# DongSky/few-shot-vit

Hardware: AMD Instinct MI355X
Metric: episodes_per_sec_5way_5shot_visformer_s (higher is better)
Workload: dtype bf16; 1 GPU; BASELINE configs[1]: Visformer-S (visformer_micro_80) miniImageNet-shaped 5-way 5-shot episodic eval, 15 query/class, 80x80 fp32 NCHW episodes resident in HBM, procedural weights + calibrated BN; images_per_episode=100, encoder_chunk_images=12800, distinct_episode_batches=16, parallelism=episode-parallel x1, one all-reduce of accuracy stats, ranks_seen=1, per_rank_eps=4439.9

## Files before the change

### few-shot-vit_amd/csrc/mlp_rows.hip

```cpp
#include <stdlib.h>

#include <type_traits>

#include "kernels.h"
#include "lds_dma.h"

namespace FSVIT_NS {

typedef __attribute__((ext_vector_type(16))) float f32x16;

namespace {

constexpr int MR_NST = 4;
constexpr int mr_slot_frags(int C) { return C == 384 ? 24 : 32; }
constexpr int MR_NW = 4;
constexpr int MR_FD = 6;
constexpr int MR_LDS_MAX = 160 * 1024;
using yes_t = std::integral_constant<bool, true>;
using no_t = std::integral_constant<bool, false>;

template <int N> __device__ __forceinline__ void mr_wait_loads(u32x4* a) {
  static_assert(N % 4 == 0 && N >= 4, "groups of 4");
  asm volatile("s_waitcnt vmcnt(0)" : "+v"(a[0]), "+v"(a[1]), "+v"(a[2]), "+v"(a[3]) :: "memory");
#pragma unroll
  for (int o = 4; o < N; o += 4) asm volatile("" : "+v"(a[o]), "+v"(a[o + 1]), "+v"(a[o + 2]), "+v"(a[o + 3]) :: "memory");
}
__device__ __forceinline__ void mfma32_v(u32x4 a, u32x4 b, f32x16& c) {
  asm volatile(FSVIT_MFMA_32x32x16 " %0, %1, %2, %0" : "+v"(c) : "v"(a), "v"(b));
}
__device__ __forceinline__ void mfma32_a(u32x4 a, u32x4 b, f32x16& c) {
  asm volatile(FSVIT_MFMA_32x32x16 " %0, %1, %2, %0" : "+a"(c) : "v"(a), "v"(b));
}
__device__ __forceinline__ void mfma32_v_z(u32x4 a, u32x4 b, f32x16& d) {
  asm volatile(FSVIT_MFMA_32x32x16 " %0, %1, %2, 0" : "=&v"(d) : "v"(a), "v"(b));
}
__device__ __forceinline__ void mfma32_a_z(u32x4 a, u32x4 b, f32x16& d) {
  asm volatile(FSVIT_MFMA_32x32x16 " %0, %1, %2, 0" : "=a"(d) : "v"(a), "v"(b));
}
__device__ __forceinline__ void mfma32_a_zero(f32x16& c) {
  const u32x4 z = {0u, 0u, 0u, 0u};
  asm volatile("s_nop 7\n\t" FSVIT_MFMA_32x32x16 " %0, %1, %1, 0" : "=a"(c) : "v"(z));
}

#define LGR_ST_MOD ""
#define LGR_LD_MOD ""
__device__ __forceinline__ void mr_gstore16(void* p, u32x4 v) {
  asm volatile("global_store_dwordx4 %0, %1, off" LGR_ST_MOD :: "v"(p), "v"(v) : "memory");
}
__device__ __forceinline__ u32x4 mr_gload16s(const void* p) {
  u32x4 v;
  asm volatile("global_load_dwordx4 %0, %1, off" LGR_LD_MOD : "=v"(v) : "v"(p) : "memory");
  return v;
}

__device__ __forceinline__ void xhalf_swap(float& a, float& b) {
  asm volatile("s_nop 1\n\tv_permlane32_swap_b32 %0, %1" : "+v"(a), "+v"(b));
}
__device__ __forceinline__ float xhalf_max(float v) {
  float a = v, b = v;
  xhalf_swap(a, b);
  return fmaxf(a, b);
}
__device__ __forceinline__ float xhalf_sum(float v) {
  float a = v, b = v;
  xhalf_swap(a, b);
  return a + b;
}

template <int NKS, int C> __device__ __forceinline__ void mr_layernorm_rows(u32x4 (&xr)[NKS], const float eps) {
  float s4[4] = {0.f, 0.f, 0.f, 0.f};
#pragma unroll
  for (int s = 0; s < NKS; ++s) {
    const bf16x8 v = __builtin_bit_cast(bf16x8, xr[s]);
#pragma unroll
    for (int e = 0; e < 8; ++e) s4[e & 3] += (float)v[e];
  }
  float sum = (s4[0] + s4[1]) + (s4[2] + s4[3]);
  sum += __shfl_xor(sum, 32);
  const float mean = sum * (1.0f / C);
#pragma unroll
  for (int o = 0; o < NKS; o += 4) asm volatile("" : "+v"(xr[o]), "+v"(xr[o + 1]), "+v"(xr[o + 2]), "+v"(xr[o + 3]));
  float q4[4] = {0.f, 0.f, 0.f, 0.f};
#pragma unroll
  for (int s = 0; s < NKS; ++s) {
    const bf16x8 v = __builtin_bit_cast(bf16x8, xr[s]);
#pragma unroll
    for (int e = 0; e < 8; ++e) { const float d = (float)v[e] - mean; q4[e & 3] = fmaf(d, d, q4[e & 3]); }
  }
  float sq = (q4[0] + q4[1]) + (q4[2] + q4[3]);
  sq += __shfl_xor(sq, 32);
  const float rstd = rsqrtf(sq * (1.0f / C) + eps);
  const float nmr = -mean * rstd;
#pragma unroll
  for (int o = 0; o < NKS; o += 4) asm volatile("" : "+v"(xr[o]), "+v"(xr[o + 1]), "+v"(xr[o + 2]), "+v"(xr[o + 3]));
#pragma unroll
  for (int s = 0; s < NKS; ++s) {
    const bf16x8 v = __builtin_bit_cast(bf16x8, xr[s]);
    u32x4 o;
#pragma unroll
    for (int e = 0; e < 4; ++e) o[e] = pk2(fmaf((float)v[2 * e], rstd, nmr), fmaf((float)v[2 * e + 1], rstd, nmr));
// ... 107 lines not shown

template <int C, int HID, int RB, int KC, bool LN>
__global__ __launch_bounds__(256, 1) void mlp_rows_kernel(const bf16* __restrict__ X, bf16* __restrict__ Y, const unsigned char* __restrict__ wimg,
                                                          const float* __restrict__ b1img, const float* __restrict__ b2, const bf16* __restrict__ CTX,
                                                          const float* __restrict__ bproj, const float ln_eps, const int M, const int n_tiles) {
  using G = mlp_rows_geom<C, HID, LN>;
  constexpr int NCT = C / 32, NKS = C / 16, NCH = HID / 32;
  constexpr int SLF = G::SLF, MR_SLOT = G::SLOT;
  constexpr int PW = SLF / MR_NW, WSH = PW * 1024;
  constexpr int SL = RB * NKS;
  constexpr int PKS = KC / 16, PFR = PKS * NCT;
  constexpr int PSLOTS = (PFR + SLF - 1) / SLF;
  static_assert(KC % 16 == 0, "whole k-steps");
  constexpr int PPC = 2 * NKS / SLF;
  constexpr int BM = MR_NW * 32 * RB;
  constexpr int FD = MR_FD;
  static_assert((SL == 32 || (SL == 24 && RB == 1)) && 2 * NKS == PPC * SLF && (PPC == 1 || PPC == 2), "register budget: <= 128 x + 256 y VGPRs");
  static_assert(!LN || (KC > 0 && RB == 1), "the LayerNorm variant continues from the proj prologue");
  static_assert(NCH % 2 == 0, "the hidden-chunk loop runs bodies in pairs behind a fixed head and tail: an even number of 32-wide chunks");
  extern __shared__ __attribute__((aligned(16))) unsigned char smem[];
  float* const b1tab = reinterpret_cast<float*>(smem + G::OFF_B1);
  float* const bptab = reinterpret_cast<float*>(smem + G::OFF_BP);
  float* const b2tab = bptab + C;
  unsigned char* const gtab = smem + G::OFF_GTAB;

  const int t = threadIdx.x, lane = t & 63;
  const int wave = __builtin_amdgcn_readfirstlane(t >> 6);
  const int r = lane & 31, kh = lane >> 5;
  const unsigned lds0 = lds_addr(smem);
  const unsigned voff = (unsigned)(wave * WSH + lane * 16);
  if ((int)blockIdx.x >= n_tiles) return;

  for (int i = t; i < HID; i += MR_NW * 64) b1tab[i] = b1img[i];
  if constexpr (LN)
    for (int i = t; i < C; i += MR_NW * 64) { bptab[i] = bproj[i]; b2tab[i] = b2[i]; }
  if constexpr (gelu_tab::ON) gelu_tab::fill(gtab, t, MR_NW * 64);
  const unsigned tabc = __builtin_amdgcn_readfirstlane(lds_addr(gtab) + 2u * gelu_tab::TN);
  asm volatile("s_waitcnt vmcnt(0) lgkmcnt(0)" ::: "memory");

  int issue_img = 0, issue_slot = 0;
  auto issue = [&]() {
    dma_n<PW>(voff, wimg + (size_t)issue_img * MR_SLOT, lds0 + issue_slot * MR_SLOT + wave * WSH);
    issue_img = issue_img == PSLOTS + NCH * PPC - 1 ? 0 : issue_img + 1;
    issue_slot = issue_slot == MR_NST - 1 ? 0 : issue_slot + 1;
  };
#pragma unroll
  for (int i = 0; i < MR_NST - 1; ++i) issue();
  int slot = 0;
  bool first = true;
  auto ring_wait = [&]() {
    asm volatile("s_waitcnt vmcnt(%0)" :: "n"(PW) : "memory");
    bar();
  };
  auto ring_sync = [&]() {
    ring_wait();
    issue();
  };
  auto issue1 = [&](int piece) {
    dma1(voff + piece * 1024, wimg + (size_t)issue_img * MR_SLOT, lds0 + issue_slot * MR_SLOT + wave * WSH + piece * 1024);
    if (piece == PW - 1) {
      issue_img = issue_img == PSLOTS + NCH * PPC - 1 ? 0 : issue_img + 1;
      issue_slot = issue_slot == MR_NST - 1 ? 0 : issue_slot + 1;
    }
  };
  auto next_slot = [&]() { slot = slot == MR_NST - 1 ? 0 : slot + 1; };

  u32x4 idf[2] = {{0u, 0u, 0u, 0u}, {0u, 0u, 0u, 0u}};
  if constexpr (LN) {
    const int ch = 16 * ((r >> 2) & 1) + 4 * (r >> 3) + (r & 3);
#pragma unroll
    for (int q = 0; q < 2; ++q)
#pragma unroll
      for (int e = 0; e < 4; ++e)
        idf[q][e] = pk2(ch == 16 * kh + 8 * q + 2 * e ? 1.0f : 0.0f, ch == 16 * kh + 8 * q + 2 * e + 1 ? 1.0f : 0.0f);
  }
  for (int tile = blockIdx.x; tile < n_tiles; tile += gridDim.x) {
    bool mok[RB];
    size_t rowoff[RB];
    int mrow[RB];
    u32x4 xr[RB][NKS];
#pragma unroll
    for (int rb = 0; rb < RB; ++rb) {
      const int m = tile * BM + (wave * RB + rb) * 32 + r;
      mok[rb] = m < M;
      mrow[rb] = mok[rb] ? m : M - 1;
      rowoff[rb] = (size_t)mrow[rb] * C + 16 * kh;
    }
    auto load_x = [&]() {
#pragma unroll
      for (int rb = 0; rb < RB; ++rb)
#pragma unroll
        for (int s = 0; s < NKS; ++s) xr[rb][s] = gload16(X + rowoff[rb] + 32 * (s >> 1) + 8 * (s & 1));
      mr_wait_loads<RB * NKS>(&xr[0][0]);
    };
    f32x16 yacc[RB][NCT];
    auto yacc_settle = [&]() {
      f32x16* yf = &yacc[0][0];
      static_assert(RB * NCT == 16 || RB * NCT == 12, "operand list");
      if constexpr (RB * NCT == 16)
        asm volatile("s_nop 15\n\ts_nop 3"
                     : "+a"(yf[0]), "+a"(yf[1]), "+a"(yf[2]), "+a"(yf[3]), "+a"(yf[4]), "+a"(yf[5]), "+a"(yf[6]), "+a"(yf[7]),
                       "+a"(yf[8]), "+a"(yf[9]), "+a"(yf[10]), "+a"(yf[11]), "+a"(yf[12]), "+a"(yf[13]), "+a"(yf[14]), "+a"(yf[15]));
      else
        asm volatile("s_nop 15\n\ts_nop 3"
                     : "+a"(yf[0]), "+a"(yf[1]), "+a"(yf[2]), "+a"(yf[3]), "+a"(yf[4]), "+a"(yf[5]), "+a"(yf[6]), "+a"(yf[7]),
                       "+a"(yf[8]), "+a"(yf[9]), "+a"(yf[10]), "+a"(yf[11]));
    };
    if constexpr (KC > 0) {
      u32x4 cr[RB][PKS];
#pragma unroll
      for (int rb = 0; rb < RB; ++rb)
#pragma unroll
        for (int ks = 0; ks < PKS; ++ks) cr[rb][ks] = gload16(CTX + (size_t)mrow[rb] * KC + 16 * ks + 8 * kh);
      mr_wait_loads<RB * PKS>(&cr[0][0]);
      if (first) { bar(); first = false; }
#pragma unroll
      for (int rb = 0; rb < RB; ++rb)
#pragma unroll
        for (int ct = 0; ct < NCT; ++ct) mfma32_a_zero(yacc[rb][ct]);
#pragma unroll
      for (int ps = 0; ps < PSLOTS; ++ps) {
        ring_sync();
        const unsigned char* sp = smem + slot * MR_SLOT + lane * 16;
        u32x4 fr[FD];
#pragma unroll
        for (int i = 0; i < FD; ++i) fr[i] = *reinterpret_cast<const u32x4*>(sp + i * 1024);
        __builtin_amdgcn_sched_barrier(0);
#pragma unroll
        for (int fi = 0; fi < SLF; ++fi) {
          const int g = ps * SLF + fi, ks = g / NCT, ct = g % NCT;
          if (g < PFR) {
#pragma unroll
            for (int rb = 0; rb < RB; ++rb) mfma32_a(fr[fi % FD], cr[rb][ks < PKS ? ks : 0], yacc[rb][ct]);
          }
          if (fi + FD < SLF && g + FD < PFR) fr[fi % FD] = *reinterpret_cast<const u32x4*>(sp + (fi + FD) * 1024);
          __builtin_amdgcn_sched_barrier(0);
        }
        next_slot();
      }
      load_x();
      yacc_settle();
#pragma unroll
      for (int rb = 0; rb < RB; ++rb)
#pragma unroll
        for (int ct = 0; ct < NCT; ++ct)
#pragma unroll
          for (int q = 0; q < 2; ++q) {
            const bf16x8 xv = __builtin_bit_cast(bf16x8, xr[rb][2 * ct + q]);
            float pb[8] = {0.f, 0.f, 0.f, 0.f, 0.f, 0.f, 0.f, 0.f};
            if constexpr (LN) {
              const f32x4 b0 = *reinterpret_cast<const f32x4*>(bptab + 32 * ct + 16 * kh + 8 * q);
              const f32x4 b1 = *reinterpret_cast<const f32x4*>(bptab + 32 * ct + 16 * kh + 8 * q + 4);
#pragma unroll
              for (int e = 0; e < 4; ++e) { pb[e] = b0[e]; pb[4 + e] = b1[e]; }
            }
            u32x4 o;
#pragma unroll
            for (int e = 0; e < 4; ++e) {
              float a0 = yacc[rb][ct][8 * q + 2 * e] + (float)xv[2 * e], a1 = yacc[rb][ct][8 * q + 2 * e + 1] + (float)xv[2 * e + 1];
              if constexpr (LN) { a0 += pb[2 * e]; a1 += pb[2 * e + 1]; }
              o[e] = pk2(a0, a1);
            }
            xr[rb][2 * ct + q] = o;
          }
    } else {
      load_x();
      if (first) { bar(); first = false; }
    }
    if constexpr (LN) {
#pragma unroll
      for (int o = 0; o + 4 < NKS; o += 4) asm volatile("" : "+v"(xr[0][o]), "+v"(xr[0][o + 1]), "+v"(xr[0][o + 2]), "+v"(xr[0][o + 3]) :: "memory");
      asm volatile("s_nop 7" : "+v"(xr[0][NKS - 4]), "+v"(xr[0][NKS - 3]), "+v"(xr[0][NKS - 2]), "+v"(xr[0][NKS - 1]), "+v"(idf[0]), "+v"(idf[1]) :: "memory");
#pragma unroll
      for (int ct = 0; ct < NCT; ++ct) {
        mfma32_a_z(idf[0], xr[0][2 * ct], yacc[0][ct]);
        mfma32_a(idf[1], xr[0][2 * ct + 1], yacc[0][ct]);
      }
      mr_layernorm_rows<NKS, C>(xr[0], ln_eps);
    } else {
#pragma unroll
      for (int rb = 0; rb < RB; ++rb)
#pragma unroll
        for (int ct = 0; ct < NCT; ++ct) mfma32_a_zero(yacc[rb][ct]);
    }

    f32x16 hacc[RB];
    u32x4 hpA[RB][2], hpB[RB][2];
    bool half = false;
    auto begin_group = [&]() -> const unsigned char* {
      unsigned a;
      if (PPC == 2) {
        ring_wait();
        a = slot * MR_SLOT + lane * 16;
// ... 107 lines not shown
          if (rb == RB - 1 && f + FD < NKS) fr[f % FD] = *reinterpret_cast<const u32x4*>(sp + foff2(f + FD));
          refill(m);
          if (m == 0 && GE) {
            if constexpr (RB == 2) asm volatile("s_nop 15\n\ts_nop 3" : "+v"(hacc[0]), "+v"(hacc[RB - 1]));
            else asm volatile("s_nop 15\n\ts_nop 3" : "+v"(hacc[0]));
          }
          if (GE) gelu_slot(m, hp_cur);
          if (G1 && m == SL - 4) bias_init(0, jn);
          __builtin_amdgcn_sched_barrier(0);
        }
      } else if (GE) {
        if constexpr (RB == 2) asm volatile("s_nop 15\n\ts_nop 3" : "+v"(hacc[0]), "+v"(hacc[RB - 1]));
        else asm volatile("s_nop 15\n\ts_nop 3" : "+v"(hacc[0]));
#pragma unroll
        for (int m = 0; m < SL; ++m) gelu_slot(m, hp_cur);
        if (G1) bias_init(0, jn);
        __builtin_amdgcn_sched_barrier(0);
      }
      if (G1) {
        const unsigned char* sp = begin_group();
#pragma unroll
        for (int i = 0; i < FD; ++i) fr[i] = *reinterpret_cast<const u32x4*>(sp + foff1(i));
        __builtin_amdgcn_sched_barrier(0);
#pragma unroll
        for (int i = 0; i < SL; ++i) {
          const int rb = RB == 2 ? i / NKS : 0, s = RB == 2 ? i % NKS : i;
          mfma32_v(fr[i % FD], xr[rb][s], hacc[rb]);
          if (i + FD < SL) fr[i % FD] = *reinterpret_cast<const u32x4*>(sp + foff1(i + FD));
          refill(i);
          if (GE) gelu_slot(SL + i, hp_cur);
          if (RB == 2 && i == NKS - 2) bias_init(1, jn);
          __builtin_amdgcn_sched_barrier(0);
        }
      } else if (GE) {
#pragma unroll
        for (int m = SL; m <= G_LAST; ++m) gelu_slot(m, hp_cur);
        __builtin_amdgcn_sched_barrier(0);
      }
    };

    bias_init(0, 0);
    body(no_t{}, no_t{}, yes_t{}, 0, hpA, hpA);
    body(no_t{}, yes_t{}, yes_t{}, 1, hpB, hpA);
#pragma unroll 1
    for (int j = 1; j < NCH - 1; j += 2) {
      body(yes_t{}, yes_t{}, yes_t{}, j + 1, hpA, hpB);
      body(yes_t{}, yes_t{}, yes_t{}, j + 2, hpB, hpA);
    }
    body(yes_t{}, yes_t{}, no_t{}, 0, hpA, hpB);
    if constexpr (RB == 2) asm volatile("s_nop 7" : "+v"(hpB[0][0]), "+v"(hpB[0][1]), "+v"(hpB[1][0]), "+v"(hpB[1][1]));
    else asm volatile("s_nop 7" : "+v"(hpB[0][0]), "+v"(hpB[0][1]));
    body(yes_t{}, no_t{}, no_t{}, 0, hpB, hpB);

    yacc_settle();
#pragma unroll
    for (int rb = 0; rb < RB; ++rb)
#pragma unroll
      for (int ct = 0; ct < NCT; ++ct) {
#pragma unroll
        for (int q = 0; q < 2; ++q) {
          const bf16x8 xv = __builtin_bit_cast(bf16x8, xr[rb][2 * ct + q]);
          bf16x8 o;
          if constexpr (LN) {
            const f32x4 b0 = *reinterpret_cast<const f32x4*>(b2tab + 32 * ct + 16 * kh + 8 * q);
            const f32x4 b1 = *reinterpret_cast<const f32x4*>(b2tab + 32 * ct + 16 * kh + 8 * q + 4);
#pragma unroll
            for (int e = 0; e < 8; ++e) o[e] = (bf16)(yacc[rb][ct][8 * q + e] + (e < 4 ? b0[e & 3] : b1[e & 3]));
          } else {
#pragma unroll
            for (int e = 0; e < 8; ++e) {
              float v = yacc[rb][ct][8 * q + e] + (float)xv[e];
              if (b2) v += b2[32 * ct + 16 * kh + 8 * q + e];
              o[e] = (bf16)v;
            }
          }
          if (mok[rb]) *reinterpret_cast<bf16x8*>(Y + rowoff[rb] + 32 * ct + 8 * q) = o;
        }
      }
  }
  asm volatile("s_waitcnt vmcnt(0)" ::: "memory");
}

#ifndef LGR_OCC
#define LGR_OCC 2
#endif
template <int C, bool LN, int SPC, int NST, bool GATHER = false>
__global__ __launch_bounds__(256, LGR_OCC) void ln_gemm_rows_kernel(const bf16* __restrict__ X, bf16* __restrict__ Y, const unsigned char* __restrict__ wimg,
                                                              const float* __restrict__ bias, const float ln_eps, const int M, const int N,
                                                              const int n_tiles, const int gH = 0, const float* __restrict__ pos = nullptr) {
  using G = gemm_rows_geom<C, SPC, NST>;
  constexpr int NKS = G::NKS, SLF = G::SLF, SLOT = G::SLOT, PW = SLF / MR_NW, WSH = PW * 1024, FD = 4, LAG = (NST - 3) * PW;
  extern __shared__ __attribute__((aligned(16))) unsigned char smem[];
  float* const btab = reinterpret_cast<float*>(smem + G::OFF_BIAS);
  const int t = threadIdx.x, lane = t & 63;
  const int wave = __builtin_amdgcn_readfirstlane(t >> 6);
  const int r = lane & 31, kh = lane >> 5;
  const unsigned lds0 = lds_addr(smem);
  const unsigned voff = (unsigned)(wave * WSH + lane * 16);
  const int nch = N / 32, n_img = nch * SPC;
  if ((int)blockIdx.x >= n_tiles) return;
  for (int i = t; i < N; i += MR_NW * 64) btab[i] = bias ? bias[i] : 0.0f;
  asm volatile("s_waitcnt vmcnt(0) lgkmcnt(0)" ::: "memory");

  int issue_img = 0, issue_slot = 0, slot = 0;
  auto issue = [&]() {
    dma_n<PW>(voff, wimg + (size_t)issue_img * SLOT, lds0 + issue_slot * SLOT + wave * WSH);
// ... 660 lines not shown
```

### few-shot-vit_amd/csrc/qkv_attn.hip

```cpp
#include <stdlib.h>

#include "lds_dma.h"
#include "kernels.h"

namespace FSVIT_NS {

namespace qa {
constexpr int C = 256, HEADS = 6, HDP = 48;
constexpr int NCT = HDP / 16, NKS = C / 32;
constexpr int NW = 8, IMGS = 2, WPI = NW / IMGS;
constexpr int TT = 2, TOK = WPI * TT * 16;
constexpr int TOKK = 112, NKT = TOKK / 16;
constexpr int FRAGS = NCT * NKS, SLOT = FRAGS * 1024;
constexpr int NST = 4, NIMG = HEADS * 3;
constexpr int PPW = FRAGS / NW;
constexpr int KS = 128 + 32;
constexpr int VS = TOK * 2 + 16;
constexpr int OFF_K = NST * SLOT, OFF_V = OFF_K + IMGS * TOKK * KS, OFF_B = OFF_V + IMGS * HDP * VS;
static_assert(OFF_B + 3 * HEADS * HDP * 4 <= 160 * 1024, "LDS budget");
constexpr int LDS_BYTES = OFF_B + 3 * HEADS * HDP * 4;
static_assert(FRAGS % NW == 0, "whole pieces per wave");
}

__global__ __launch_bounds__(qa::NW * 64) void qkv_attn_kernel(const bf16* __restrict__ X, bf16* __restrict__ CTX, const unsigned char* __restrict__ wimg,
                                                               const float* __restrict__ bias, const int B, const int S, const float scale) {
  using namespace qa;
  extern __shared__ __attribute__((aligned(16))) unsigned char smem[];
  float* const btab = reinterpret_cast<float*>(smem + OFF_B);
  const unsigned lds0 = lds_addr(smem);
  const int t = threadIdx.x, lane = t & 63;
  const int wave = __builtin_amdgcn_readfirstlane(t >> 6);
  const int sub = wave / WPI, tokbase = (wave % WPI) * (TT * 16);
  unsigned char* const Ks = smem + OFF_K + sub * (TOKK * KS);
  unsigned char* const Vt = smem + OFF_V + sub * (HDP * VS);
  const int m = lane & 15, lq = lane >> 4;
  const u32x4 zero4 = {0u, 0u, 0u, 0u};
  const int n_pass = (B + IMGS - 1) / IMGS;
  if ((int)blockIdx.x >= n_pass) return;

  for (int i = t; i < 3 * HEADS * HDP; i += NW * 64) btab[i] = bias ? bias[i] : 0.0f;
  for (int i = t; i < (OFF_B - OFF_K) / 16; i += NW * 64) *reinterpret_cast<u32x4*>(smem + OFF_K + i * 16) = zero4;
  asm volatile("s_waitcnt vmcnt(0) lgkmcnt(0)" ::: "memory");

  int issue_img = 0, issue_slot = 0;
  const unsigned voff = (unsigned)(wave * PPW * 1024 + lane * 16);
  auto issue1 = [&](int piece) {
    dma1(voff + piece * 1024, wimg + (size_t)issue_img * SLOT, lds0 + issue_slot * SLOT + (wave * PPW + piece) * 1024);
    if (piece == PPW - 1) {
      issue_img = issue_img == NIMG - 1 ? 0 : issue_img + 1;
      issue_slot = issue_slot == NST - 1 ? 0 : issue_slot + 1;
    }
  };
#pragma unroll
  for (int i = 0; i < NST - 1; ++i)
#pragma unroll
    for (int pc = 0; pc < PPW; ++pc) issue1(pc);
  int slot = 0;
  asm volatile("s_barrier" ::: "memory");

  const float sscale = scale * 1.44269504088896340736f;

  u32x4 xr[TT][NKS];
  auto load_x = [&](int pass) {
    const int img = pass * IMGS + sub;
#pragma unroll
    for (int tt = 0; tt < TT; ++tt) {
      const int tok = tokbase + 16 * tt + m;
      const bool ok = img < B && tok < S;
      const bf16* src = X + ((size_t)(img < B ? img : B - 1) * S + (tok < S ? tok : S - 1)) * C + lq * 8;
#pragma unroll
      for (int ks = 0; ks < NKS; ++ks) xr[tt][ks] = ok ? gload16(src + ks * 32) : zero4;
    }
  };
  load_x(blockIdx.x);

  for (int pass = blockIdx.x; pass < n_pass; pass += gridDim.x) {
    const int img = pass * IMGS + sub;
    asm volatile("s_waitcnt vmcnt(0)" : "+v"(xr[0][0]), "+v"(xr[0][1]), "+v"(xr[0][2]), "+v"(xr[0][3]) :: "memory");
    asm volatile("" : "+v"(xr[0][4]), "+v"(xr[0][5]), "+v"(xr[0][6]), "+v"(xr[0][7]) :: "memory");
    asm volatile("" : "+v"(xr[1][0]), "+v"(xr[1][1]), "+v"(xr[1][2]), "+v"(xr[1][3]) :: "memory");
    asm volatile("" : "+v"(xr[1][4]), "+v"(xr[1][5]), "+v"(xr[1][6]), "+v"(xr[1][7]) :: "memory");
    bf16* const obase = CTX + (size_t)img * S * (HEADS * HDP);
    u32x2 pend[TT][NCT];
    int pend_h = -1;
    auto flush_ctx = [&]() {
      if (pend_h < 0) return;
#pragma unroll
      for (int tt = 0; tt < TT; ++tt) {
        const int q = tokbase + 16 * tt + m;
        if (img < B && q < S) {
#pragma unroll
          for (int dt = 0; dt < NCT; ++dt) *reinterpret_cast<u32x2*>(obase + (size_t)q * (HEADS * HDP) + pend_h * HDP + dt * 16 + lq * 4) = pend[tt][dt];
        }
      }
      pend_h = -1;
    };

#pragma unroll 1
    for (int h = 0; h < HEADS; ++h) {
      u32x4 qf[TT][2];
#pragma unroll
      for (int pi = 0; pi < 3; ++pi) {
        const int p = pi == 2 ? 0 : pi + 1;
        asm volatile("s_waitcnt vmcnt(%0) lgkmcnt(0)" :: "n"(PPW) : "memory");
        asm volatile("s_barrier" ::: "memory");
        if (pi == 2) flush_ctx();
        __builtin_amdgcn_sched_barrier(0);
        const unsigned char* sp = smem + slot * SLOT + lane * 16;
        slot = slot == NST - 1 ? 0 : slot + 1;
        const float* bp = btab + (p * HEADS + h) * HDP;
        f32x4 acc[NCT][TT];
#pragma unroll
        for (int c = 0; c < NCT; ++c)
#pragma unroll
          for (int tt = 0; tt < TT; ++tt) {
            if (p < 2) acc[c][tt] = *reinterpret_cast<const f32x4*>(bp + 16 * c + 4 * lq);
            else { const float bv = bp[16 * c + m]; acc[c][tt] = f32x4{bv, bv, bv, bv}; }
          }
#pragma unroll
        for (int ks = 0; ks < NKS; ++ks) {
#pragma unroll
          for (int c = 0; c < NCT; ++c) {
            const u32x4 wf = *reinterpret_cast<const u32x4*>(sp + (ks * NCT + c) * 1024);
#pragma unroll
            for (int tt = 0; tt < TT; ++tt)
              acc[c][tt] = p < 2 ? mma_chunk<bf16>(wf, xr[tt][ks], acc[c][tt]) : mma_chunk<bf16>(xr[tt][ks], wf, acc[c][tt]);
          }
          if (ks % 3 == 0 && ks / 3 < PPW) issue1(ks / 3);
        }
#pragma unroll
        for (int tt = 0; tt < TT; ++tt) {
          const int tok = tokbase + 16 * tt + m;
          if (p == 0) {
            qf[tt][0] = u32x4{pk2(acc[0][tt][0], acc[0][tt][1]), pk2(acc[0][tt][2], acc[0][tt][3]),
                              pk2(acc[1][tt][0], acc[1][tt][1]), pk2(acc[1][tt][2], acc[1][tt][3])};
            qf[tt][1] = u32x4{pk2(acc[2][tt][0], acc[2][tt][1]), pk2(acc[2][tt][2], acc[2][tt][3]), 0u, 0u};
          } else if (tokbase + 16 * tt >= TOKK) {
          } else if (p == 1) {
            const int ksw = 16 * (lq ^ ((m >> 2) & 1));
            *reinterpret_cast<u32x4*>(Ks + tok * KS + ksw) = u32x4{pk2(acc[0][tt][0], acc[0][tt][1]), pk2(acc[0][tt][2], acc[0][tt][3]),
                                                                   pk2(acc[1][tt][0], acc[1][tt][1]), pk2(acc[1][tt][2], acc[1][tt][3])};
            *reinterpret_cast<u32x2*>(Ks + tok * KS + 64 + ksw) = u32x2{pk2(acc[2][tt][0], acc[2][tt][1]), pk2(acc[2][tt][2], acc[2][tt][3])};
          } else {
#pragma unroll
            for (int c = 0; c < NCT; ++c) {
              const u32x2 o = {pk2(acc[c][tt][0], acc[c][tt][1]), pk2(acc[c][tt][2], acc[c][tt][3])};
              *reinterpret_cast<u32x2*>(Vt + (16 * c + m) * VS + (tokbase + 16 * tt + 4 * lq) * 2) = o;
            }
          }
        }
      }
      if (h == HEADS - 1 && pass + (int)gridDim.x < n_pass) load_x(pass + gridDim.x);

      {
        f32x4 sc[TT][NKT];
#pragma unroll
        for (int kt = 0; kt < NKT; ++kt) {
          const unsigned char* ka = Ks + (kt * 16 + m) * KS + 16 * (lq ^ ((m >> 2) & 1));
          const u32x4 k0 = *reinterpret_cast<const u32x4*>(ka), k1 = *reinterpret_cast<const u32x4*>(ka + 64);
#pragma unroll
          for (int tt = 0; tt < TT; ++tt) {
            f32x4 a = {0.f, 0.f, 0.f, 0.f};
            a = mma_chunk<bf16>(k0, qf[tt][0], a);
            sc[tt][kt] = mma_chunk<bf16>(k1, qf[tt][1], a);
          }
        }
        float inv[TT];
#pragma unroll
        for (int tt = 0; tt < TT; ++tt) {
          float mx = -INFINITY;
#pragma unroll
          for (int kt = 0; kt < NKT; ++kt) {
            if (kt * 16 + 16 > S) {
#pragma unroll
              for (int r = 0; r < 4; ++r)
                if (kt * 16 + lq * 4 + r >= S) sc[tt][kt][r] = -INFINITY;
            }
#pragma unroll
            for (int r = 0; r < 4; ++r) mx = fmaxf(mx, sc[tt][kt][r]);
          }
          mx = fmaxf(mx, __shfl_xor(mx, 16, 64));
          mx = fmaxf(mx, __shfl_xor(mx, 32, 64));
          const float mxs = mx * sscale;
          float sum = 0.f;
#pragma unroll
          for (int kt = 0; kt < NKT; ++kt)
#pragma unroll
            for (int r = 0; r < 4; ++r) {
              const float e = __builtin_amdgcn_exp2f(fmaf(sc[tt][kt][r], sscale, -mxs));
              sc[tt][kt][r] = e;
              sum += e;
            }
          sum += __shfl_xor(sum, 16, 64);
          sum += __shfl_xor(sum, 32, 64);
          inv[tt] = 1.0f / sum;
        }
        pend_h = h;
        constexpr int NPC = (NKT + 1) / 2;
        u32x4 pb[TT][NPC];
#pragma unroll
        for (int tt = 0; tt < TT; ++tt)
#pragma unroll
          for (int kc = 0; kc < NPC; ++kc) {
            const bool two = 2 * kc + 1 < NKT;
            pb[tt][kc] = u32x4{pk2(sc[tt][2 * kc][0], sc[tt][2 * kc][1]), pk2(sc[tt][2 * kc][2], sc[tt][2 * kc][3]),
                               two ? pk2(sc[tt][two ? 2 * kc + 1 : 0][0], sc[tt][two ? 2 * kc + 1 : 0][1]) : 0u,
                               two ? pk2(sc[tt][two ? 2 * kc + 1 : 0][2], sc[tt][two ? 2 * kc + 1 : 0][3]) : 0u};
          }
#pragma unroll
        for (int dt = 0; dt < NCT; ++dt) {
          f32x4 a[TT];
#pragma unroll
          for (int tt = 0; tt < TT; ++tt) a[tt] = f32x4{0.f, 0.f, 0.f, 0.f};
          const unsigned char* va = Vt + (dt * 16 + m) * VS;
#pragma unroll
          for (int kc = 0; kc < NPC; ++kc) {
            const u32x2 v0 = *reinterpret_cast<const u32x2*>(va + (32 * kc + lq * 4) * 2);
            const u32x2 v1 = *reinterpret_cast<const u32x2*>(va + (32 * kc + 16 + lq * 4) * 2);
            const u32x4 vf = {v0[0], v0[1], v1[0], v1[1]};
#pragma unroll
            for (int tt = 0; tt < TT; ++tt) a[tt] = mma_chunk<bf16>(vf, pb[tt][kc], a[tt]);
          }
#pragma unroll
          for (int tt = 0; tt < TT; ++tt) {
            const f32x4 o = a[tt] * inv[tt];
            pend[tt][dt] = u32x2{pk2(o[0], o[1]), pk2(o[2], o[3])};
          }
        }
      }
    }
    flush_ctx();
  }
  asm volatile("s_waitcnt vmcnt(0)" ::: "memory");
}

__global__ void qkv_attn_pack_kernel(const bf16* __restrict__ w, int kw, bf16* __restrict__ img) {
  using namespace qa;
  const long idx = (long)blockIdx.x * blockDim.x + threadIdx.x;
  if (idx >= (long)NIMG * FRAGS * 512) return;
  const int e8 = (int)idx & 7, lane = (int)(idx >> 3) & 63, f = (int)(idx >> 9) % FRAGS, n = (int)(idx >> 9) / FRAGS;
  const int h = n / 3, p = (n % 3 + 1) % 3, ks = f / NCT, c = f % NCT, m = lane & 15, lq = lane >> 4;
  img[idx] = w[(size_t)((p * HEADS + h) * HDP + 16 * c + m) * kw + 32 * ks + 8 * lq + e8];
}

bool qkv_attn_supported(int dtype, int C, int heads, int hdp, int S) {
  constexpr int on = 1;
  return on && dtype == 1 && C == qa::C && heads == qa::HEADS && hdp == qa::HDP && S >= 1 && S <= qa::TOKK;
}
size_t qkv_attn_image_bytes() { return (size_t)qa::NIMG * qa::SLOT; }

int launch_qkv_attn_pack(const void* w, int kw, void* img, hipStream_t s) {
  const long n = (long)qa::NIMG * qa::FRAGS * 512;
  hipLaunchKernelGGL(qkv_attn_pack_kernel, dim3((unsigned)((n + 255) / 256)), dim3(256), 0, s, (const bf16*)w, kw, (bf16*)img);
  return (int)hipGetLastError();
}

int launch_qkv_attn(const void* x, void* ctx, const void* wimg, const float* bias, int B, int S, float scale, hipStream_t s) {
  if (B <= 0) return 0;
  {
    hipError_t e = hipFuncSetAttribute((const void*)qkv_attn_kernel, hipFuncAttributeMaxDynamicSharedMemorySize, qa::LDS_BYTES);
    if (e != hipSuccess) return (int)e;
  }
  const int n_pass = (B + qa::IMGS - 1) / qa::IMGS;
  const int grid = n_pass < 256 ? n_pass : 256;
  hipLaunchKernelGGL(qkv_attn_kernel, dim3(grid), dim3(qa::NW * 64), qa::LDS_BYTES, s, (const bf16*)x, (bf16*)ctx, (const unsigned char*)wimg, bias, B, S,
                     scale);
  return (int)hipGetLastError();
}

}
```

Before: 4436 episodes/s.

## Split and prefetch context loads across tiles and overlap residual loads with projection

Splits the per-tile context-row loads into two halves. The first half is prefetched for the next tile at the end of the current tile, and the second half is waited on only when the MFMA loop first needs it. Residual X loads are interleaved into the projection MFMA loop instead of being issued and drained afterwards, with counted vmcnt waits layered on top of the weight-ring DMA counts. This aims to hide global-load latency behind matrix work, at the cost of more live registers and fragile wait-count bookkeeping.

```diff
diff --git a/few-shot-vit_amd/csrc/mlp_rows.hip b/few-shot-vit_amd/csrc/mlp_rows.hip
--- a/few-shot-vit_amd/csrc/mlp_rows.hip
+++ b/few-shot-vit_amd/csrc/mlp_rows.hip
@@ -25,6 +25,12 @@
 #pragma unroll
   for (int o = 4; o < N; o += 4) asm volatile("" : "+v"(a[o]), "+v"(a[o + 1]), "+v"(a[o + 2]), "+v"(a[o + 3]) :: "memory");
 }
+template <int CNT, int N> __device__ __forceinline__ void mr_wait_loads_n(u32x4* a) {
+  static_assert(CNT >= 0 && CNT <= 63 && N >= 1, "6-bit vmcnt");
+  asm volatile("s_waitcnt vmcnt(%1)" : "+v"(a[0]) : "n"(CNT) : "memory");
+#pragma unroll
+  for (int o = 1; o < N; ++o) asm volatile("" : "+v"(a[o]) :: "memory");
+}
 __device__ __forceinline__ void mfma32_v(u32x4 a, u32x4 b, f32x16& c) {
   asm volatile(FSVIT_MFMA_32x32x16 " %0, %1, %2, %0" : "+v"(c) : "v"(a), "v"(b));
 }
@@ -46,6 +52,12 @@
 #define LGR_LD_MOD ""
 __device__ __forceinline__ void mr_gstore16(void* p, u32x4 v) {
   asm volatile("global_store_dwordx4 %0, %1, off" LGR_ST_MOD :: "v"(p), "v"(v) : "memory");
+}
+template <int OFF> __device__ __forceinline__ u32x4 mr_gload16o(const void* p) {
+  static_assert(OFF >= 0 && OFF < 4096, "13-bit signed offset field");
+  u32x4 v;
+  asm volatile("global_load_dwordx4 %0, %1, off offset:%2" : "=v"(v) : "v"(p), "n"(OFF) : "memory");
+  return v;
 }
 __device__ __forceinline__ u32x4 mr_gload16s(const void* p) {
   u32x4 v;
@@ -259,10 +271,6 @@
     asm volatile("s_waitcnt vmcnt(%0)" :: "n"(PW) : "memory");
     bar();
   };
-  auto ring_sync = [&]() {
-    ring_wait();
-    issue();
-  };
   auto issue1 = [&](int piece) {
     dma1(voff + piece * 1024, wimg + (size_t)issue_img * MR_SLOT, lds0 + issue_slot * MR_SLOT + wave * WSH + piece * 1024);
     if (piece == PW - 1) {
@@ -280,6 +288,21 @@
 #pragma unroll
       for (int e = 0; e < 4; ++e)
         idf[q][e] = pk2(ch == 16 * kh + 8 * q + 2 * e ? 1.0f : 0.0f, ch == 16 * kh + 8 * q + 2 * e + 1 ? 1.0f : 0.0f);
+  }
+  constexpr bool CARRY = KC > 0 && !LN;
+  constexpr int CH1 = KC > 0 ? KC / 32 : 1;
+  u32x4 crA[RB][CH1];
+  auto load_ctx_a = [&](const int tile_) {
+    static_for<RB>([&](auto rbc) {
+      constexpr int rb = decltype(rbc)::value;
+      const int m = tile_ * BM + (wave * RB + rb) * 32 + r;
+      const bf16* const cb = CTX + (size_t)(m < M ? m : M - 1) * KC + 8 * kh;
+      static_for<CH1>([&](auto ksc) { crA[rb][decltype(ksc)::value] = mr_gload16o<32 * decltype(ksc)::value>(cb); });
+    });
+  };
+  if constexpr (CARRY) {
+    load_ctx_a(blockIdx.x);
+    mr_wait_loads_n<0, RB * CH1>(&crA[0][0]);
   }
   for (int tile = blockIdx.x; tile < n_tiles; tile += gridDim.x) {
     bool mok[RB];
@@ -314,38 +337,59 @@
                        "+a"(yf[8]), "+a"(yf[9]), "+a"(yf[10]), "+a"(yf[11]));
     };
     if constexpr (KC > 0) {
-      u32x4 cr[RB][PKS];
+      constexpr int H1 = PKS / 2, H2 = PKS - H1, GH = H1 * NCT, PB = GH / SLF, FB = GH % SLF;
+      constexpr int NLB = RB * H2, NX = RB * NKS, XPER = (NX + SLF - FB - 1) / (SLF - FB);
+      static_assert(PB >= 2 && PB + 2 <= PSLOTS - 1, "half B lands by ring wait 2; the two counted waits behind the x loads are proj ring waits");
+      static_assert(PW + NLB <= 63 && PW + NX <= 63, "6-bit vmcnt");
+      static_assert(H1 == CH1, "the carried half");
+      u32x4 crB[RB][H2];
+      const bf16* cbase[RB];
+#pragma unroll
+      for (int rb = 0; rb < RB; ++rb) cbase[rb] = CTX + (size_t)mrow[rb] * KC + 8 * kh;
+      if constexpr (!CARRY) load_ctx_a(tile);
+      static_for<RB * H2>([&](auto ic) {
+        constexpr int rb = decltype(ic)::value / H2, ks = decltype(ic)::value % H2;
+        crB[rb][ks] = mr_gload16o<32 * (H1 + ks)>(cbase[rb]);
+      });
+      mr_wait_loads_n<NLB, RB * H1>(&crA[0][0]);
+      if (first) { bar(); first = false; }
 #pragma unroll
       for (int rb = 0; rb < RB; ++rb)
 #pragma unroll
-        for (int ks = 0; ks < PKS; ++ks) cr[rb][ks] = gload16(CTX + (size_t)mrow[rb] * KC + 16 * ks + 8 * kh);
-      mr_wait_loads<RB * PKS>(&cr[0][0]);
-      if (first) { bar(); first = false; }
-#pragma unroll
-      for (int rb = 0; rb < RB; ++rb)
-#pragma unroll
         for (int ct = 0; ct < NCT; ++ct) mfma32_a_zero(yacc[rb][ct]);
-#pragma unroll
-      for (int ps = 0; ps < PSLOTS; ++ps) {
-        ring_sync();
+      static_for<PSLOTS>([&](auto psc) {
+        constexpr int ps = decltype(psc)::value;
+        constexpr int EXTRA = ps < 2 ? NLB : (ps == PB + 1 || ps == PB + 2 ? NX : 0);
+        asm volatile("s_waitcnt vmcnt(%0)" :: "n"(PW + EXTRA) : "memory");
+        bar();
+        issue();
         const unsigned char* sp = smem + slot * MR_SLOT + lane * 16;
         u32x4 fr[FD];
 #pragma unroll
         for (int i = 0; i < FD; ++i) fr[i] = *reinterpret_cast<const u32x4*>(sp + i * 1024);
         __builtin_amdgcn_sched_barrier(0);
-#pragma unroll
-        for (int fi = 0; fi < SLF; ++fi) {
-          const int g = ps * SLF + fi, ks = g / NCT, ct = g % NCT;
-          if (g < PFR) {
-#pragma unroll
-            for (int rb = 0; rb < RB; ++rb) mfma32_a(fr[fi % FD], cr[rb][ks < PKS ? ks : 0], yacc[rb][ct]);
+        static_for<SLF>([&](auto fic) {
+          constexpr int fi = decltype(fic)::value, g = ps * SLF + fi, ks = g / NCT, ct = g % NCT;
+          if constexpr (g == GH) mr_wait_loads_n<PW, NLB>(&crB[0][0]);
+          if constexpr (g < PFR) {
+#pragma unroll
+            for (int rb = 0; rb < RB; ++rb) {
+              if constexpr (ks < H1) mfma32_a(fr[fi % FD], crA[rb][ks], yacc[rb][ct]);
+              else mfma32_a(fr[fi % FD], crB[rb][ks - H1], yacc[rb][ct]);
+            }
           }
-          if (fi + FD < SLF && g + FD < PFR) fr[fi % FD] = *reinterpret_cast<const u32x4*>(sp + (fi + FD) * 1024);
+          if constexpr (fi + FD < SLF && g + FD < PFR) fr[fi % FD] = *reinterpret_cast<const u32x4*>(sp + (fi + FD) * 1024);
+          if constexpr (ps == PB && fi >= FB) {
+            static_for<XPER>([&](auto kc) {
+              constexpr int i = (fi - FB) * XPER + decltype(kc)::value, rb = i / NKS, xs = i % NKS;
+              if constexpr (i < NX) xr[rb][xs] = mr_gload16o<2 * (32 * (xs >> 1) + 8 * (xs & 1))>(X + rowoff[rb]);
+            });
+          }
           __builtin_amdgcn_sched_barrier(0);
-        }
+        });
         next_slot();
-      }
-      load_x();
+      });
+      mr_wait_loads_n<2 * PW, NX>(&xr[0][0]);
       yacc_settle();
 #pragma unroll
       for (int rb = 0; rb < RB; ++rb)
@@ -559,6 +603,7 @@
     else asm volatile("s_nop 7" : "+v"(hpB[0][0]), "+v"(hpB[0][1]));
     body(yes_t{}, no_t{}, no_t{}, 0, hpB, hpB);
 
+    if constexpr (CARRY) load_ctx_a(tile + gridDim.x);
     yacc_settle();
 #pragma unroll
     for (int rb = 0; rb < RB; ++rb)
```

Measured after the change: 4465 episodes/s (median of 6 runs). Within noise of the previous version (+0.7%).

## Software-pipeline attention of previous head into QKV projection GEMMs

Applied to the files above, without the earlier changes.

Restructures the fused QKV+attention kernel so the softmax and PV work for head h-1 is interleaved inside the K and V projection GEMM loops for head h, with Q computed last and the attention finished after the loop. It also double-buffers the weight-fragment LDS reads within each GEMM and templates the kernel on S/16 so the key-masking bounds are compile-time. The aim is to hide attention latency behind MFMA projection work and cut LDS stalls, at the cost of higher register pressure and more complex barrier and waitcnt sequencing.

```diff
diff --git a/few-shot-vit_amd/csrc/qkv_attn.hip b/few-shot-vit_amd/csrc/qkv_attn.hip
--- a/few-shot-vit_amd/csrc/qkv_attn.hip
+++ b/few-shot-vit_amd/csrc/qkv_attn.hip
@@ -22,6 +22,7 @@
 static_assert(FRAGS % NW == 0, "whole pieces per wave");
 }
 
+template <int KTM>
 __global__ __launch_bounds__(qa::NW * 64) void qkv_attn_kernel(const bf16* __restrict__ X, bf16* __restrict__ CTX, const unsigned char* __restrict__ wimg,
                                                                const float* __restrict__ bias, const int B, const int S, const float scale) {
   using namespace qa;
@@ -74,163 +75,226 @@
   };
   load_x(blockIdx.x);
 
+  constexpr int NPC = (NKT + 1) / 2;
+  u32x4 qf[TT][2];
+  f32x4 sc[TT][NKT];
+  u32x4 pb[TT][NPC];
+  u32x2 pend[TT][NCT];
+  float mxs[TT], sum[TT], inv[TT];
+  bf16* pobase = CTX;
+  int ph = 0;
+  bool pok = false;
+#pragma unroll
+  for (int tt = 0; tt < TT; ++tt) qf[tt][0] = qf[tt][1] = zero4;
+
+  auto att_scores = [&]() {
+#pragma unroll
+    for (int kt = 0; kt < NKT; ++kt) {
+      const unsigned char* ka = Ks + (kt * 16 + m) * KS + 16 * (lq ^ ((m >> 2) & 1));
+      const u32x4 k0 = *reinterpret_cast<const u32x4*>(ka), k1 = *reinterpret_cast<const u32x4*>(ka + 64);
+#pragma unroll
+      for (int tt = 0; tt < TT; ++tt) {
+        f32x4 a = {0.f, 0.f, 0.f, 0.f};
+        a = mma_chunk<bf16>(k0, qf[tt][0], a);
+        sc[tt][kt] = mma_chunk<bf16>(k1, qf[tt][1], a);
+      }
+    }
+  };
+  auto att_max = [&](int tt) {
+    float mx = -INFINITY;
+#pragma unroll
+    for (int kt = 0; kt < NKT; ++kt) {
+      if (kt >= KTM) {
+#pragma unroll
+        for (int r = 0; r < 4; ++r)
+          if (kt > KTM || kt * 16 + lq * 4 + r >= S) sc[tt][kt][r] = -INFINITY;
+      }
+#pragma unroll
+      for (int r = 0; r < 4; ++r) mx = fmaxf(mx, sc[tt][kt][r]);
+    }
+    mx = fmaxf(mx, __shfl_xor(mx, 16, 64));
+    mx = fmaxf(mx, __shfl_xor(mx, 32, 64));
+    mxs[tt] = mx * sscale;
+    sum[tt] = 0.f;
+  };
+  auto att_exp = [&](int tt, int kt0, int kt1) {
+#pragma unroll
+    for (int kt = kt0; kt < kt1; ++kt)
+#pragma unroll
+      for (int r = 0; r < 4; ++r) {
+        const float e = __builtin_amdgcn_exp2f(fmaf(sc[tt][kt][r], sscale, -mxs[tt]));
+        sc[tt][kt][r] = e;
+        sum[tt] += e;
+      }
+  };
+  auto att_fin = [&](int tt) {
+    float sm = sum[tt];
+    sm += __shfl_xor(sm, 16, 64);
+    sm += __shfl_xor(sm, 32, 64);
+    inv[tt] = 1.0f / sm;
+#pragma unroll
+    for (int kc = 0; kc < NPC; ++kc) {
+      const bool two = 2 * kc + 1 < NKT;
+      pb[tt][kc] = u32x4{pk2(sc[tt][2 * kc][0], sc[tt][2 * kc][1]), pk2(sc[tt][2 * kc][2], sc[tt][2 * kc][3]),
+                         two ? pk2(sc[tt][two ? 2 * kc + 1 : 0][0], sc[tt][two ? 2 * kc + 1 : 0][1]) : 0u,
+                         two ? pk2(sc[tt][two ? 2 * kc + 1 : 0][2], sc[tt][two ? 2 * kc + 1 : 0][3]) : 0u};
+    }
+  };
+  auto att_pv = [&](int dt) {
+    f32x4 a[TT];
+#pragma unroll
+    for (int tt = 0; tt < TT; ++tt) a[tt] = f32x4{0.f, 0.f, 0.f, 0.f};
+    const unsigned char* va = Vt + (dt * 16 + m) * VS;
+#pragma unroll
+    for (int kc = 0; kc < NPC; ++kc) {
+      const u32x2 v0 = *reinterpret_cast<const u32x2*>(va + (32 * kc + lq * 4) * 2);
+      const u32x2 v1 = *reinterpret_cast<const u32x2*>(va + (32 * kc + 16 + lq * 4) * 2);
+      const u32x4 vf = {v0[0], v0[1], v1[0], v1[1]};
+#pragma unroll
+      for (int tt = 0; tt < TT; ++tt) a[tt] = mma_chunk<bf16>(vf, pb[tt][kc], a[tt]);
+    }
+#pragma unroll
+    for (int tt = 0; tt < TT; ++tt) {
+      const f32x4 o = a[tt] * inv[tt];
+      pend[tt][dt] = u32x2{pk2(o[0], o[1]), pk2(o[2], o[3])};
+    }
+  };
+  auto flush_ctx = [&]() {
+#pragma unroll
+    for (int tt = 0; tt < TT; ++tt) {
+      const int q = tokbase + 16 * tt + m;
+      if (pok && q < S) {
+#pragma unroll
+        for (int dt = 0; dt < NCT; ++dt) *reinterpret_cast<u32x2*>(pobase + (size_t)q * (HEADS * HDP) + ph * HDP + dt * 16 + lq * 4) = pend[tt][dt];
+      }
+    }
+  };
+  auto gemm_part = [&](auto P, int h, f32x4 (&acc)[NCT][TT], auto&& hook) {
+    constexpr int p = decltype(P)::value;
+    const unsigned char* sp = smem + slot * SLOT + lane * 16;
+    slot = slot == NST - 1 ? 0 : slot + 1;
+    const float* bp = btab + (p * HEADS + h) * HDP;
+#pragma unroll
+    for (int c = 0; c < NCT; ++c)
+#pragma unroll
+      for (int tt = 0; tt < TT; ++tt) {
+        if (p < 2) acc[c][tt] = *reinterpret_cast<const f32x4*>(bp + 16 * c + 4 * lq);
+        else { const float bv = bp[16 * c + m]; acc[c][tt] = f32x4{bv, bv, bv, bv}; }
+      }
+    u32x4 wf[NCT], wfn[NCT];
+#pragma unroll
+    for (int c = 0; c < NCT; ++c) wf[c] = *reinterpret_cast<const u32x4*>(sp + c * 1024);
+    static_for<NKS>([&](auto KSI) {
+      constexpr int ks = decltype(KSI)::value;
+      if constexpr (ks + 1 < NKS) {
+#pragma unroll
+        for (int c = 0; c < NCT; ++c) wfn[c] = *reinterpret_cast<const u32x4*>(sp + ((ks + 1) * NCT + c) * 1024);
+      }
+      __builtin_amdgcn_sched_barrier(0x406);
+#pragma unroll
+      for (int c = 0; c < NCT; ++c)
+#pragma unroll
+        for (int tt = 0; tt < TT; ++tt)
+          acc[c][tt] = p < 2 ? mma_chunk<bf16>(wf[c], xr[tt][ks], acc[c][tt]) : mma_chunk<bf16>(xr[tt][ks], wf[c], acc[c][tt]);
+      if constexpr (ks % 3 == 0 && ks / 3 < PPW) issue1(ks / 3);
+      hook(KSI);
+      if constexpr (ks + 1 < NKS) {
+#pragma unroll
+        for (int c = 0; c < NCT; ++c) wf[c] = wfn[c];
+      }
+    });
+  };
+
   for (int pass = blockIdx.x; pass < n_pass; pass += gridDim.x) {
     const int img = pass * IMGS + sub;
-    asm volatile("s_waitcnt vmcnt(0)" : "+v"(xr[0][0]), "+v"(xr[0][1]), "+v"(xr[0][2]), "+v"(xr[0][3]) :: "memory");
-    asm volatile("" : "+v"(xr[0][4]), "+v"(xr[0][5]), "+v"(xr[0][6]), "+v"(xr[0][7]) :: "memory");
-    asm volatile("" : "+v"(xr[1][0]), "+v"(xr[1][1]), "+v"(xr[1][2]), "+v"(xr[1][3]) :: "memory");
-    asm volatile("" : "+v"(xr[1][4]), "+v"(xr[1][5]), "+v"(xr[1][6]), "+v"(xr[1][7]) :: "memory");
     bf16* const obase = CTX + (size_t)img * S * (HEADS * HDP);
-    u32x2 pend[TT][NCT];
-    int pend_h = -1;
-    auto flush_ctx = [&]() {
-      if (pend_h < 0) return;
-#pragma unroll
-      for (int tt = 0; tt < TT; ++tt) {
-        const int q = tokbase + 16 * tt + m;
-        if (img < B && q < S) {
-#pragma unroll
-          for (int dt = 0; dt < NCT; ++dt) *reinterpret_cast<u32x2*>(obase + (size_t)q * (HEADS * HDP) + pend_h * HDP + dt * 16 + lq * 4) = pend[tt][dt];
-        }
-      }
-      pend_h = -1;
-    };
 
 #pragma unroll 1
     for (int h = 0; h < HEADS; ++h) {
-      u32x4 qf[TT][2];
-#pragma unroll
-      for (int pi = 0; pi < 3; ++pi) {
-        const int p = pi == 2 ? 0 : pi + 1;
-        asm volatile("s_waitcnt vmcnt(%0) lgkmcnt(0)" :: "n"(PPW) : "memory");
-        asm volatile("s_barrier" ::: "memory");
-        if (pi == 2) flush_ctx();
-        __builtin_amdgcn_sched_barrier(0);
-        const unsigned char* sp = smem + slot * SLOT + lane * 16;
-        slot = slot == NST - 1 ? 0 : slot + 1;
-        const float* bp = btab + (p * HEADS + h) * HDP;
-        f32x4 acc[NCT][TT];
-#pragma unroll
-        for (int c = 0; c < NCT; ++c)
-#pragma unroll
-          for (int tt = 0; tt < TT; ++tt) {
-            if (p < 2) acc[c][tt] = *reinterpret_cast<const f32x4*>(bp + 16 * c + 4 * lq);
-            else { const float bv = bp[16 * c + m]; acc[c][tt] = f32x4{bv, bv, bv, bv}; }
-          }
-#pragma unroll
-        for (int ks = 0; ks < NKS; ++ks) {
-#pragma unroll
-          for (int c = 0; c < NCT; ++c) {
-            const u32x4 wf = *reinterpret_cast<const u32x4*>(sp + (ks * NCT + c) * 1024);
-#pragma unroll
-            for (int tt = 0; tt < TT; ++tt)
-              acc[c][tt] = p < 2 ? mma_chunk<bf16>(wf, xr[tt][ks], acc[c][tt]) : mma_chunk<bf16>(xr[tt][ks], wf, acc[c][tt]);
-          }
-          if (ks % 3 == 0 && ks / 3 < PPW) issue1(ks / 3);
+      f32x4 acc[NCT][TT];
+      if (h == 0) asm volatile("s_waitcnt vmcnt(%0) lgkmcnt(0)" :: "n"(PPW + TT * NKS) : "memory");
+      else asm volatile("s_waitcnt vmcnt(%0) lgkmcnt(0)" :: "n"(PPW) : "memory");
+      asm volatile("s_barrier" ::: "memory");
+      __builtin_amdgcn_sched_barrier(0);
+      att_scores();
+      if (h == 0) {
+        asm volatile("s_waitcnt vmcnt(0)" : "+v"(xr[0][0]), "+v"(xr[0][1]), "+v"(xr[0][2]), "+v"(xr[0][3]) :: "memory");
+        asm volatile("" : "+v"(xr[0][4]), "+v"(xr[0][5]), "+v"(xr[0][6]), "+v"(xr[0][7]) :: "memory");
+        asm volatile("" : "+v"(xr[1][0]), "+v"(xr[1][1]), "+v"(xr[1][2]), "+v"(xr[1][3]) :: "memory");
+        asm volatile("" : "+v"(xr[1][4]), "+v"(xr[1][5]), "+v"(xr[1][6]), "+v"(xr[1][7]) :: "memory");
+      }
+      gemm_part(std::integral_constant<int, 1>{}, h, acc, [&](auto KSI) {
+        constexpr int ks = decltype(KSI)::value;
+        if constexpr (ks == 0) att_max(0);
+        if constexpr (ks == 1) att_exp(0, 0, 4);
+        if constexpr (ks == 2) { att_exp(0, 4, NKT); att_fin(0); }
+        if constexpr (ks == 3) att_max(1);
+        if constexpr (ks == 4) att_exp(1, 0, 4);
+        if constexpr (ks == 5) { att_exp(1, 4, NKT); att_fin(1); }
+      });
+      u32x4 kp0[TT];
+      u32x2 kp1[TT];
+#pragma unroll
+      for (int tt = 0; tt < TT; ++tt) {
+        kp0[tt] = u32x4{pk2(acc[0][tt][0], acc[0][tt][1]), pk2(acc[0][tt][2], acc[0][tt][3]), pk2(acc[1][tt][0], acc[1][tt][1]), pk2(acc[1][tt][2], acc[1][tt][3])};
+        kp1[tt] = u32x2{pk2(acc[2][tt][0], acc[2][tt][1]), pk2(acc[2][tt][2], acc[2][tt][3])};
+      }
+
+      asm volatile("s_waitcnt vmcnt(%0) lgkmcnt(0)" :: "n"(PPW) : "memory");
+      asm volatile("s_barrier" ::: "memory");
+      __builtin_amdgcn_sched_barrier(0);
+#pragma unroll
+      for (int tt = 0; tt < TT; ++tt) {
+        const int tok = tokbase + 16 * tt + m;
+        if (tokbase + 16 * tt < TOKK) {
+          const int ksw = 16 * (lq ^ ((m >> 2) & 1));
+          *reinterpret_cast<u32x4*>(Ks + tok * KS + ksw) = kp0[tt];
+          *reinterpret_cast<u32x2*>(Ks + tok * KS + 64 + ksw) = kp1[tt];
         }
-#pragma unroll
-        for (int tt = 0; tt < TT; ++tt) {
-          const int tok = tokbase + 16 * tt + m;
-          if (p == 0) {
-            qf[tt][0] = u32x4{pk2(acc[0][tt][0], acc[0][tt][1]), pk2(acc[0][tt][2], acc[0][tt][3]),
-                              pk2(acc[1][tt][0], acc[1][tt][1]), pk2(acc[1][tt][2], acc[1][tt][3])};
-            qf[tt][1] = u32x4{pk2(acc[2][tt][0], acc[2][tt][1]), pk2(acc[2][tt][2], acc[2][tt][3]), 0u, 0u};
-          } else if (tokbase + 16 * tt >= TOKK) {
-          } else if (p == 1) {
-            const int ksw = 16 * (lq ^ ((m >> 2) & 1));
-            *reinterpret_cast<u32x4*>(Ks + tok * KS + ksw) = u32x4{pk2(acc[0][tt][0], acc[0][tt][1]), pk2(acc[0][tt][2], acc[0][tt][3]),
-                                                                   pk2(acc[1][tt][0], acc[1][tt][1]), pk2(acc[1][tt][2], acc[1][tt][3])};
-            *reinterpret_cast<u32x2*>(Ks + tok * KS + 64 + ksw) = u32x2{pk2(acc[2][tt][0], acc[2][tt][1]), pk2(acc[2][tt][2], acc[2][tt][3])};
-          } else {
-#pragma unroll
-            for (int c = 0; c < NCT; ++c) {
-              const u32x2 o = {pk2(acc[c][tt][0], acc[c][tt][1]), pk2(acc[c][tt][2], acc[c][tt][3])};
-              *reinterpret_cast<u32x2*>(Vt + (16 * c + m) * VS + (tokbase + 16 * tt + 4 * lq) * 2) = o;
-            }
-          }
+      }
+      gemm_part(std::integral_constant<int, 2>{}, h, acc, [&](auto KSI) {
+        constexpr int ks = decltype(KSI)::value;
+        if constexpr (ks % 3 == 0) att_pv(ks / 3);
+      });
+      u32x2 vp[TT][NCT];
+#pragma unroll
+      for (int tt = 0; tt < TT; ++tt)
+#pragma unroll
+        for (int c = 0; c < NCT; ++c) vp[tt][c] = u32x2{pk2(acc[c][tt][0], acc[c][tt][1]), pk2(acc[c][tt][2], acc[c][tt][3])};
+
+      asm volatile("s_waitcnt vmcnt(%0) lgkmcnt(0)" :: "n"(PPW) : "memory");
+      asm volatile("s_barrier" ::: "memory");
+      flush_ctx();
+      __builtin_amdgcn_sched_barrier(0);
+#pragma unroll
+      for (int tt = 0; tt < TT; ++tt)
+        if (tokbase + 16 * tt < TOKK) {
+#pragma unroll
+          for (int c = 0; c < NCT; ++c) *reinterpret_cast<u32x2*>(Vt + (16 * c + m) * VS + (tokbase + 16 * tt + 4 * lq) * 2) = vp[tt][c];
         }
-      }
+      gemm_part(std::integral_constant<int, 0>{}, h, acc, [&](auto) {});
+#pragma unroll
+      for (int tt = 0; tt < TT; ++tt) {
+        qf[tt][0] = u32x4{pk2(acc[0][tt][0], acc[0][tt][1]), pk2(acc[0][tt][2], acc[0][tt][3]), pk2(acc[1][tt][0], acc[1][tt][1]), pk2(acc[1][tt][2], acc[1][tt][3])};
+        qf[tt][1] = u32x4{pk2(acc[2][tt][0], acc[2][tt][1]), pk2(acc[2][tt][2], acc[2][tt][3]), 0u, 0u};
+      }
+      pobase = obase, ph = h, pok = img < B;
       if (h == HEADS - 1 && pass + (int)gridDim.x < n_pass) load_x(pass + gridDim.x);
-
-      {
-        f32x4 sc[TT][NKT];
-#pragma unroll
-        for (int kt = 0; kt < NKT; ++kt) {
-          const unsigned char* ka = Ks + (kt * 16 + m) * KS + 16 * (lq ^ ((m >> 2) & 1));
-          const u32x4 k0 = *reinterpret_cast<const u32x4*>(ka), k1 = *reinterpret_cast<const u32x4*>(ka + 64);
-#pragma unroll
-          for (int tt = 0; tt < TT; ++tt) {
-            f32x4 a = {0.f, 0.f, 0.f, 0.f};
-            a = mma_chunk<bf16>(k0, qf[tt][0], a);
-            sc[tt][kt] = mma_chunk<bf16>(k1, qf[tt][1], a);
-          }
-        }
-        float inv[TT];
-#pragma unroll
-        for (int tt = 0; tt < TT; ++tt) {
-          float mx = -INFINITY;
-#pragma unroll
-          for (int kt = 0; kt < NKT; ++kt) {
-            if (kt * 16 + 16 > S) {
-#pragma unroll
-              for (int r = 0; r < 4; ++r)
-                if (kt * 16 + lq * 4 + r >= S) sc[tt][kt][r] = -INFINITY;
-            }
-#pragma unroll
-            for (int r = 0; r < 4; ++r) mx = fmaxf(mx, sc[tt][kt][r]);
-          }
-          mx = fmaxf(mx, __shfl_xor(mx, 16, 64));
-          mx = fmaxf(mx, __shfl_xor(mx, 32, 64));
-          const float mxs = mx * sscale;
-          float sum = 0.f;
-#pragma unroll
-          for (int kt = 0; kt < NKT; ++kt)
-#pragma unroll
-            for (int r = 0; r < 4; ++r) {
-              const float e = __builtin_amdgcn_exp2f(fmaf(sc[tt][kt][r], sscale, -mxs));
-              sc[tt][kt][r] = e;
-              sum += e;
-            }
-          sum += __shfl_xor(sum, 16, 64);
-          sum += __shfl_xor(sum, 32, 64);
-          inv[tt] = 1.0f / sum;
-        }
-        pend_h = h;
-        constexpr int NPC = (NKT + 1) / 2;
-        u32x4 pb[TT][NPC];
-#pragma unroll
-        for (int tt = 0; tt < TT; ++tt)
-#pragma unroll
-          for (int kc = 0; kc < NPC; ++kc) {
-            const bool two = 2 * kc + 1 < NKT;
-            pb[tt][kc] = u32x4{pk2(sc[tt][2 * kc][0], sc[tt][2 * kc][1]), pk2(sc[tt][2 * kc][2], sc[tt][2 * kc][3]),
-                               two ? pk2(sc[tt][two ? 2 * kc + 1 : 0][0], sc[tt][two ? 2 * kc + 1 : 0][1]) : 0u,
-                               two ? pk2(sc[tt][two ? 2 * kc + 1 : 0][2], sc[tt][two ? 2 * kc + 1 : 0][3]) : 0u};
-          }
-#pragma unroll
-        for (int dt = 0; dt < NCT; ++dt) {
-          f32x4 a[TT];
-#pragma unroll
-          for (int tt = 0; tt < TT; ++tt) a[tt] = f32x4{0.f, 0.f, 0.f, 0.f};
-          const unsigned char* va = Vt + (dt * 16 + m) * VS;
-#pragma unroll
-          for (int kc = 0; kc < NPC; ++kc) {
-            const u32x2 v0 = *reinterpret_cast<const u32x2*>(va + (32 * kc + lq * 4) * 2);
-            const u32x2 v1 = *reinterpret_cast<const u32x2*>(va + (32 * kc + 16 + lq * 4) * 2);
-            const u32x4 vf = {v0[0], v0[1], v1[0], v1[1]};
-#pragma unroll
-            for (int tt = 0; tt < TT; ++tt) a[tt] = mma_chunk<bf16>(vf, pb[tt][kc], a[tt]);
-          }
-#pragma unroll
-          for (int tt = 0; tt < TT; ++tt) {
-            const f32x4 o = a[tt] * inv[tt];
-            pend[tt][dt] = u32x2{pk2(o[0], o[1]), pk2(o[2], o[3])};
-          }
-        }
-      }
-    }
-    flush_ctx();
+    }
   }
+  asm volatile("s_waitcnt lgkmcnt(0)" ::: "memory");
+  asm volatile("s_barrier" ::: "memory");
+  __builtin_amdgcn_sched_barrier(0);
+  att_scores();
+#pragma unroll
+  for (int tt = 0; tt < TT; ++tt) {
+    att_max(tt);
+    att_exp(tt, 0, NKT);
+    att_fin(tt);
+  }
+#pragma unroll
+  for (int dt = 0; dt < NCT; ++dt) att_pv(dt);
+  flush_ctx();
   asm volatile("s_waitcnt vmcnt(0)" ::: "memory");
 }
 
@@ -257,15 +321,25 @@
 
 int launch_qkv_attn(const void* x, void* ctx, const void* wimg, const float* bias, int B, int S, float scale, hipStream_t s) {
   if (B <= 0) return 0;
-  {
-    hipError_t e = hipFuncSetAttribute((const void*)qkv_attn_kernel, hipFuncAttributeMaxDynamicSharedMemorySize, qa::LDS_BYTES);
-    if (e != hipSuccess) return (int)e;
-  }
+  if (S < 1 || S > qa::TOKK) return (int)hipErrorInvalidValue;
   const int n_pass = (B + qa::IMGS - 1) / qa::IMGS;
   const int grid = n_pass < 256 ? n_pass : 256;
-  hipLaunchKernelGGL(qkv_attn_kernel, dim3(grid), dim3(qa::NW * 64), qa::LDS_BYTES, s, (const bf16*)x, (bf16*)ctx, (const unsigned char*)wimg, bias, B, S,
-                     scale);
-  return (int)hipGetLastError();
-}
-
-}
+  auto go = [&](auto kernel) {
+    hipError_t e = hipFuncSetAttribute((const void*)kernel, hipFuncAttributeMaxDynamicSharedMemorySize, qa::LDS_BYTES);
+    if (e != hipSuccess) return (int)e;
+    hipLaunchKernelGGL(kernel, dim3(grid), dim3(qa::NW * 64), qa::LDS_BYTES, s, (const bf16*)x, (bf16*)ctx, (const unsigned char*)wimg, bias, B, S, scale);
+    return (int)hipGetLastError();
+  };
+  switch (S / 16) {
+    case 0: return go(qkv_attn_kernel<0>);
+    case 1: return go(qkv_attn_kernel<1>);
+    case 2: return go(qkv_attn_kernel<2>);
+    case 3: return go(qkv_attn_kernel<3>);
+    case 4: return go(qkv_attn_kernel<4>);
+    case 5: return go(qkv_attn_kernel<5>);
+    case 6: return go(qkv_attn_kernel<6>);
+    default: return go(qkv_attn_kernel<7>);
+  }
+}
+
+}
```

Result: no change. 4429 episodes/s before, 4455 episodes/s after (median of 6 runs) (+0.6%).
